# thedonutfactory/rs-tfhe

Hardware: AMD Instinct MI355X
Metric: gate-bootstraps/sec (hom_nand, SECURITY_128_BIT) (higher is better)
Workload: dtype f64

## Files before the change

rs-tfhe_amd/csrc/key_switch_mfma.hpp:

```cpp
#pragma once
#include <hip/hip_runtime.h>
#include <stdint.h>

#include <type_traits>

#include "experiment.hpp"

namespace tfhe {

#ifndef TFHE_KM_FRAGS
#define TFHE_KM_FRAGS 1
#endif
#ifndef TFHE_KM_COLBLOCKS
#define TFHE_KM_COLBLOCKS 2
#endif
constexpr int kKmWaves = 4;
constexpr int kKmFrags = TFHE_KM_FRAGS;
constexpr int kKmRows = 32 * kKmFrags * kKmWaves;
#ifndef TFHE_KM_SLOTS
#define TFHE_KM_SLOTS 4
#endif
constexpr int kKmSlots = TFHE_KM_SLOTS;
constexpr int kKmAhead = kKmSlots - 1;
constexpr int kKmAbBytes = 32 * kKmFrags * 16 * 4;
constexpr int kKmAbQ = kKmAbBytes / 256;
constexpr int kKmColBlocks = TFHE_KM_COLBLOCKS;
constexpr int kKmMaxTiles = 12 / kKmFrags;

__host__ __device__ constexpr int ks_mfma_tpw(int nt) { return (nt + kKmWaves - 1) / kKmWaves; }
__host__ __device__ constexpr int ks_mfma_slot_bytes(int nt) { return ks_mfma_tpw(nt) * kKmWaves * 1024; }
__host__ __device__ constexpr size_t ks_mfma_lds_bytes(int nt) {
  return (size_t)kKmSlots * ks_mfma_slot_bytes(nt) + (size_t)kKmWaves * 2 * kKmAbBytes + (size_t)kKmWaves * 256;
}
__host__ __device__ __forceinline__ int ks_mfma_total_tiles(int n) { return (n + 1 + 31) / 32; }
__host__ __device__ __forceinline__ int ks_mfma_tiles(int n) { return (ks_mfma_total_tiles(n) + kKmColBlocks - 1) / kKmColBlocks; }
__host__ __device__ __forceinline__ int ks_mfma_block_tiles(int n, int cb) {
  const int tiles = ks_mfma_total_tiles(n);
  return tiles / kKmColBlocks + (cb < tiles % kKmColBlocks ? 1 : 0);
}
__host__ __device__ __forceinline__ int ks_mfma_block_first(int n, int cb) {
  const int tiles = ks_mfma_total_tiles(n), base = tiles / kKmColBlocks, rem = tiles % kKmColBlocks;
  return cb * base + (cb < rem ? cb : rem);
}
__host__ __device__ __forceinline__ size_t ks_mfma_key_bytes(int n, int t) {
  return (size_t)4 * (64 * 2 * t) * ks_mfma_total_tiles(n) * 1024;
}
constexpr size_t kKmKeyTailPad = 64 * 1024;

__host__ __device__ __forceinline__ uint32_t ks_plane_byte(uint32_t w, int p) {
  uint32_t s = 0;
  for (int q = 0; q <= p; ++q) {
    s = w & 0xFFu;
    const uint32_t sext = (s & 0x80u) ? (s | 0xFFFFFF00u) : s;
    w = (w - sext) >> 8;
  }
  return s;
}

__global__ void k_ksk_planes(const uint32_t *__restrict__ eng, unsigned char *__restrict__ out, int n, int t,
                             size_t chunks) {
  const size_t idx = (size_t)blockIdx.x * blockDim.x + threadIdx.x;
  if (idx >= chunks) return;
  const int lane = (int)(idx & 63);
  size_t r = idx >> 6;
  const int S = 64 * 2 * t, tiles = ks_mfma_total_tiles(n);
  const size_t per_plane = (size_t)S * tiles;
  const int p = (int)(r / per_plane);
  r -= (size_t)p * per_plane;
  int cb = 0;
  while (cb + 1 < kKmColBlocks && r >= (size_t)S * ks_mfma_block_first(n, cb + 1)) ++cb;
  r -= (size_t)S * ks_mfma_block_first(n, cb);
  const int nt = ks_mfma_block_tiles(n, cb);
  const int s = (int)(r / (size_t)nt), c = (int)(r % (size_t)nt);
  const int col = (ks_mfma_block_first(n, cb) + c) * 32 + (lane & 31), kb = lane >> 5;
  const int blk = s / (2 * t), u = s % (2 * t), j = u >> 1, hh = u & 1;
  const int rw = (n + 1 + 3) & ~3;
  uint32_t o[4];
#pragma unroll
  for (int cc = 0; cc < 4; ++cc) {
    const int i = 16 * blk + 8 * hh + 4 * kb + cc;
    uint32_t d = 0;
#pragma unroll
    for (int k = 0; k < 4; ++k) {
      const size_t row = ((size_t)i * t + j) * 4 + k;
      const uint32_t w = (col <= n && k != 0) ? eng[row * (size_t)rw + col] : 0u;
      d |= ks_plane_byte(w, p) << (8 * k);
    }
    o[cc] = d;
  }
  reinterpret_cast<uint4 *>(out)[idx] = make_uint4(o[0], o[1], o[2], o[3]);
}

using km_i32x4 = __attribute__((ext_vector_type(4))) int;
using km_i32x16 = __attribute__((ext_vector_type(16))) int;
using km_u32x4 = __attribute__((ext_vector_type(4))) unsigned int;

__device__ __forceinline__ void km_dma16(uint32_t voff, const void *sbase, uint32_t lds) {
  uint32_t keep;
  asm volatile(
      "s_mov_b32 %0, m0\n\t"
      "s_mov_b32 m0, %3\n\t"
      "s_nop 0\n\t"
      "global_load_lds_dwordx4 %1, %2\n\t"
      "s_mov_b32 m0, %0"
      : "=&s"(keep)
      : "v"(voff), "s"(sbase), "s"(lds)
      : "memory");
}
__device__ __forceinline__ void km_dma4(uint32_t voff, const void *sbase, uint32_t lds) {
  uint32_t keep;
  asm volatile(
      "s_mov_b32 %0, m0\n\t"
      "s_mov_b32 m0, %3\n\t"
      "s_nop 0\n\t"
      "global_load_lds_dword %1, %2\n\t"
      "s_mov_b32 m0, %0"
      : "=&s"(keep)
      : "v"(voff), "s"(sbase), "s"(lds)
      : "memory");
}

struct KmPos {
  int blk, u;
};

#ifndef TFHE_KM_XCD
#define TFHE_KM_XCD 1
#endif
template <int NT>
__global__ __launch_bounds__(64 * kKmWaves, 2) void k_key_switch_mfma(const uint32_t *__restrict__ lv1,
                                                                       const unsigned char *__restrict__ ksk8,
                                                                       int n, int t, uint32_t *__restrict__ out,
                                                                       size_t count,
                                                                       unsigned long long *clk,
                                                                       int ksplit) {
  constexpr int N = 1024, D = kKmAhead, WAVES = kKmWaves, R = kKmFrags;
  constexpr int TPW = ks_mfma_tpw(NT), SLOT = ks_mfma_slot_bytes(NT), OPS = TPW + R;
  const unsigned long long clk0 = clk ? __builtin_amdgcn_s_memtime() : 0ull;
  const unsigned long long rtc0 = clk ? __builtin_amdgcn_s_memrealtime() : 0ull;
  extern __shared__ __attribute__((aligned(16))) unsigned char km_smem[];
  const int tid = threadIdx.x, lane = tid & 63;
  const int wave = __builtin_amdgcn_readfirstlane(tid >> 6);
  const uint32_t lds_base = (uint32_t)(size_t)(__attribute__((address_space(3))) unsigned char *)km_smem;
  const uint32_t off_ab = (uint32_t)(kKmSlots * SLOT) + (uint32_t)wave * 2u * kKmAbBytes;
  const uint32_t off_dump = (uint32_t)(kKmSlots * SLOT) + (uint32_t)(WAVES * 2 * kKmAbBytes) + (uint32_t)wave * 256u;
#if TFHE_KM_XCD
  const unsigned lin = blockIdx.x + gridDim.x * (blockIdx.y + gridDim.y * blockIdx.z);
  const unsigned combos = gridDim.y * gridDim.z, combo = lin % combos, rest = lin / combos;
  const int cb = (int)(combo % gridDim.y), plane = (int)(combo / gridDim.y);
#else
  const unsigned rest = blockIdx.x;
  const int cb = blockIdx.y, plane = blockIdx.z;
#endif
  const unsigned n_rb = gridDim.x / (unsigned)ksplit;
  const int kchunk = (int)(rest / n_rb);
  const int blk0 = kchunk * (64 / ksplit);
  const size_t row0 = (size_t)(rest % n_rb) * kKmRows + (size_t)wave * (32 * R);
  const int nt_blk = ks_mfma_block_tiles(n, cb), tile0 = ks_mfma_block_first(n, cb);
  const bool full = nt_blk == NT;
  const int spb = 2 * t, S = 64 * spb;
  const uint32_t prec = 1u << (31 - 2 * t);
  const uint32_t v16 = (uint32_t)lane * 16u;
  const uint32_t v4 = (uint32_t)(((lane >> 4) * (N + 1) + (lane & 15)) * 4);
  const uint32_t *ab_row0 = lv1 + row0 * (size_t)(N + 1);

  const unsigned char *kplane = ksk8 + ((size_t)plane * ks_mfma_total_tiles(n) + (size_t)tile0) * S * 1024;
  uint32_t koff[TPW];
#pragma unroll
  for (int i = 0; i < TPW; ++i) {
    const int tile = wave + i * WAVES;
    koff[i] = (uint32_t)(tile < nt_blk ? tile : nt_blk - 1) * 1024u + v16;
  }
  const uint32_t kstride = (uint32_t)nt_blk * 1024u;
  const int steps = S / ksplit;
#pragma unroll
  for (int i = 0; i < TPW; ++i) koff[i] += (uint32_t)(blk0 * spb) * kstride;
  auto dma_key = [&](uint32_t slot) {
#pragma unroll
    for (int i = 0; i < TPW; ++i) {
      km_dma16(koff[i], kplane, slot + (uint32_t)(wave + i * WAVES) * 1024u);
      koff[i] += kstride;
    }
  };

  for (int q = 0; q < kKmAbQ; ++q) km_dma4(v4, ab_row0 + (size_t)(4 * q) * (N + 1) + 16 * blk0, lds_base + off_ab + (uint32_t)q * 256u);
  for (int d = 0; d < D; ++d) dma_key(lds_base + (uint32_t)d * SLOT);
  asm volatile("s_waitcnt vmcnt(0)" ::: "memory");
  __builtin_amdgcn_s_barrier();
  asm volatile("" ::: "memory");

  km_i32x16 acc[R][NT];
  const uint32_t a_lane = (uint32_t)((lane & 31) * 64 + (lane >> 5) * 16);
  auto read_a = [&](const KmPos &q, int f) -> km_u32x4 {
    const unsigned char *abuf = km_smem + off_ab + (uint32_t)(q.blk & 1) * kKmAbBytes + a_lane + (uint32_t)(q.u & 1) * 32u;
    return *reinterpret_cast<const km_u32x4 *>(abuf + f * (32 * 64));
  };
  auto build_a = [&](const KmPos &q, km_u32x4 w) -> km_i32x4 {
    const uint32_t sh = (uint32_t)(27 - 2 * (q.u >> 1));
    km_u32x4 a;
    a.x = 1u << (((w.x + prec) >> sh) & 0x18u);
    a.y = 1u << (((w.y + prec) >> sh) & 0x18u);
    a.z = 1u << (((w.z + prec) >> sh) & 0x18u);
    a.w = 1u << (((w.w + prec) >> sh) & 0x18u);
    return __builtin_bit_cast(km_i32x4, a);
  };
  auto make_a = [&](const KmPos &q, int f) -> km_i32x4 { return build_a(q, read_a(q, f)); };
  KmPos cur{blk0, 0};
  km_i32x4 A[R];
#pragma unroll
  for (int f = 0; f < R; ++f) A[f] = make_a(cur, f);
#ifndef TFHE_KM_PRE
#define TFHE_KM_PRE 3
#endif
  constexpr int PRE = NT < TFHE_KM_PRE ? NT : TFHE_KM_PRE;
  constexpr int H = NT / 2;
  km_i32x4 Bpre[PRE];
#pragma unroll
  for (int c = 0; c < PRE; ++c) Bpre[c] = *reinterpret_cast<const km_i32x4 *>(km_smem + v16 + c * 1024);
#pragma unroll
  for (int f = 0; f < R; ++f)
#pragma unroll
    for (int c = 0; c < NT; ++c) acc[f][c] = km_i32x16{0, 0, 0, 0, 0, 0, 0, 0, 0, 0, 0, 0, 0, 0, 0, 0};
  auto run = [&](auto full_c) {
    constexpr bool FULL = decltype(full_c)::value;
#pragma unroll 1
    for (int g = 0; g < steps; ++g) {
      const unsigned char *slot = km_smem + (uint32_t)(g % kKmSlots) * SLOT + v16;
      const unsigned char *slot_next = km_smem + (uint32_t)((g + 1) % kKmSlots) * SLOT + v16;
      km_i32x4 B[NT];
#pragma unroll
      for (int c = 0; c < PRE; ++c) B[c] = Bpre[c];
#pragma unroll
      for (int c = 0; c < H; ++c) {
        if (c + PRE < NT) B[c + PRE] = *reinterpret_cast<const km_i32x4 *>(slot + (c + PRE) * 1024);
#pragma unroll
        for (int f = 0; f < R; ++f) acc[f][c] = __builtin_amdgcn_mfma_i32_32x32x32_i8(A[f], B[c], acc[f][c], 0, 0, 0);
      }
      __builtin_amdgcn_sched_barrier(0);
      asm volatile("s_waitcnt vmcnt(%0)" ::"n"((D - 2) * OPS) : "memory");
      if (!TFHE_ABL_KM_NOBARRIER) __builtin_amdgcn_s_barrier();
      asm volatile("" ::: "memory");
      const uint32_t dslot = lds_base + (uint32_t)((g + D) % kKmSlots) * SLOT;
      const int nblk = (cur.blk + 1) & 63;
      const uint32_t nbuf = lds_base + off_ab + (uint32_t)((cur.blk + 1) & 1) * kKmAbBytes;
      const int u_now = cur.u;
      constexpr int PIECES = TPW + R + 2;
      km_i32x4 A_next[R];
      km_u32x4 Aw[R];
      auto piece = [&](int it) {
        if (it == 0) {
          if (++cur.u == spb) {
            cur.u = 0;
            cur.blk = (cur.blk + 1) & 63;
          }
#pragma unroll
          for (int f = 0; f < R; ++f) Aw[f] = read_a(cur, f);
#pragma unroll
          for (int c = 0; c < PRE; ++c) Bpre[c] = *reinterpret_cast<const km_i32x4 *>(slot_next + c * 1024);
        } else if (it == PIECES - 2) {
#pragma unroll
          for (int f = 0; f < R; ++f) A_next[f] = build_a(cur, Aw[f]);
        } else {
          const int d = it - 1 - (it > PIECES - 2 ? 1 : 0);
          if (d < TPW) {
            km_dma16(koff[d], kplane, dslot + (uint32_t)(wave + d * WAVES) * 1024u);
            koff[d] += kstride;
          } else {
            const int q0 = R * u_now + (d - TPW);
            const uint32_t *s0 = ab_row0 + (size_t)(4 * (q0 & (kKmAbQ - 1))) * (N + 1) + 16 * nblk;
            km_dma4(v4, s0, q0 < kKmAbQ ? nbuf + (uint32_t)q0 * 256u : lds_base + off_dump);
          }
        }
      };
#pragma unroll
      for (int c = H; c < NT; ++c) {
        if (c + PRE < NT) B[c + PRE] = *reinterpret_cast<const km_i32x4 *>(slot + (c + PRE) * 1024);
        if (c < NT - 1 || FULL) {
#pragma unroll
          for (int f = 0; f < R; ++f) acc[f][c] = __builtin_amdgcn_mfma_i32_32x32x32_i8(A[f], B[c], acc[f][c], 0, 0, 0);
        }
        __builtin_amdgcn_sched_barrier(0);
        if (c - H < PIECES) piece(c - H);
        __builtin_amdgcn_sched_barrier(0);
      }
#pragma unroll
      for (int it = NT - H; it < PIECES; ++it) piece(it);
#pragma unroll
      for (int f = 0; f < R; ++f) A[f] = A_next[f];
    }
  };
  if (full)
    run(std::true_type{});
  else
    run(std::false_type{});
  {
    const int sh8 = 8 * plane;
    const int row_lim = (int)(count > row0 ? (count - row0 < 32 * R ? count - row0 : 32 * R) : 0) - 4 * (lane >> 5);
    const int col_lane = tile0 * 32 + (lane & 31);
    const uint32_t lane_off = (uint32_t)((4 * (lane >> 5)) * (n + 1) + col_lane) * 4u;
    unsigned char *obase = reinterpret_cast<unsigned char *>(out + row0 * (size_t)(n + 1));
    const uint32_t row_bytes = (uint32_t)(n + 1) * 4u;
#pragma unroll
    for (int f = 0; f < R; ++f)
#pragma unroll
      for (int c = 0; c < NT; ++c) {
        const bool col_ok = col_lane + 32 * c <= n && c < nt_blk;
        const bool is_body = col_lane + 32 * c == n && plane == 0 && kchunk == 0;
#pragma unroll
        for (int e = 0; e < 16; ++e) {
          const int er = 32 * f + (e & 3) + 8 * (e >> 2);
          if (col_ok && er < row_lim) {
            uint32_t v = 0u - ((uint32_t)acc[f][c][e] << sh8);
            if (is_body) v += lv1[(row0 + (size_t)(er + 4 * (lane >> 5))) * (size_t)(N + 1) + N];
            unsigned char *uni = obase + (size_t)((uint32_t)er * row_bytes + (uint32_t)(c * 128));
            if (v) atomicAdd(reinterpret_cast<uint32_t *>(uni + lane_off), v);
          }
        }
      }
  }
  asm volatile("s_waitcnt vmcnt(0)" ::: "memory");
  if (clk && tid == 0) {
    atomicAdd(&clk[0], __builtin_amdgcn_s_memtime() - clk0);
    atomicAdd(&clk[1], __builtin_amdgcn_s_memrealtime() - rtc0);
  }
}

}
```

Measured before the change: 191,000.

## Pack three nonzero key-switch digits per K slot to cut MFMA steps

After: 191,500 (median of 6 runs). Within noise of the previous version (+0.3%).

```diff
diff --git a/rs-tfhe_amd/csrc/key_switch_mfma.hpp b/rs-tfhe_amd/csrc/key_switch_mfma.hpp
--- a/rs-tfhe_amd/csrc/key_switch_mfma.hpp
+++ b/rs-tfhe_amd/csrc/key_switch_mfma.hpp
@@ -22,15 +22,16 @@
 #endif
 constexpr int kKmSlots = TFHE_KM_SLOTS;
 constexpr int kKmAhead = kKmSlots - 1;
-constexpr int kKmAbBytes = 32 * kKmFrags * 16 * 4;
+constexpr int kKmBlocks = 32;
+constexpr int kKmAbBytes = 32 * kKmFrags * 32 * 4;
 constexpr int kKmAbQ = kKmAbBytes / 256;
 constexpr int kKmColBlocks = TFHE_KM_COLBLOCKS;
 constexpr int kKmMaxTiles = 12 / kKmFrags;
 
 __host__ __device__ constexpr int ks_mfma_tpw(int nt) { return (nt + kKmWaves - 1) / kKmWaves; }
-__host__ __device__ constexpr int ks_mfma_slot_bytes(int nt) { return ks_mfma_tpw(nt) * kKmWaves * 1024; }
+__host__ __device__ constexpr int ks_mfma_slot_bytes(int nt) { return nt * 1024; }
 __host__ __device__ constexpr size_t ks_mfma_lds_bytes(int nt) {
-  return (size_t)kKmSlots * ks_mfma_slot_bytes(nt) + (size_t)kKmWaves * 2 * kKmAbBytes + (size_t)kKmWaves * 256;
+  return (size_t)kKmSlots * ks_mfma_slot_bytes(nt) + (size_t)kKmWaves * 2 * kKmAbBytes + 1024;
 }
 __host__ __device__ __forceinline__ int ks_mfma_total_tiles(int n) { return (n + 1 + 31) / 32; }
 __host__ __device__ __forceinline__ int ks_mfma_tiles(int n) { return (ks_mfma_total_tiles(n) + kKmColBlocks - 1) / kKmColBlocks; }
@@ -42,8 +43,9 @@
   const int tiles = ks_mfma_total_tiles(n), base = tiles / kKmColBlocks, rem = tiles % kKmColBlocks;
   return cb * base + (cb < rem ? cb : rem);
 }
+__host__ __device__ __forceinline__ int ks_mfma_steps(int t) { return kKmBlocks * 3 * t; }
 __host__ __device__ __forceinline__ size_t ks_mfma_key_bytes(int n, int t) {
-  return (size_t)4 * (64 * 2 * t) * ks_mfma_total_tiles(n) * 1024;
+  return (size_t)4 * ks_mfma_steps(t) * ks_mfma_total_tiles(n) * 1024;
 }
 constexpr size_t kKmKeyTailPad = 64 * 1024;
 
@@ -63,7 +65,7 @@
   if (idx >= chunks) return;
   const int lane = (int)(idx & 63);
   size_t r = idx >> 6;
-  const int S = 64 * 2 * t, tiles = ks_mfma_total_tiles(n);
+  const int S = ks_mfma_steps(t), tiles = ks_mfma_total_tiles(n);
   const size_t per_plane = (size_t)S * tiles;
   const int p = (int)(r / per_plane);
   r -= (size_t)p * per_plane;
@@ -73,20 +75,21 @@
   const int nt = ks_mfma_block_tiles(n, cb);
   const int s = (int)(r / (size_t)nt), c = (int)(r % (size_t)nt);
   const int col = (ks_mfma_block_first(n, cb) + c) * 32 + (lane & 31), kb = lane >> 5;
-  const int blk = s / (2 * t), u = s % (2 * t), j = u >> 1, hh = u & 1;
+  const int unit = s / 3, s3 = s % 3, blk = unit / t, j = unit % t;
   const int rw = (n + 1 + 3) & ~3;
   uint32_t o[4];
 #pragma unroll
-  for (int cc = 0; cc < 4; ++cc) {
-    const int i = 16 * blk + 8 * hh + 4 * kb + cc;
-    uint32_t d = 0;
-#pragma unroll
-    for (int k = 0; k < 4; ++k) {
+  for (int d = 0; d < 4; ++d) {
+    uint32_t v = 0;
+#pragma unroll
+    for (int e = 0; e < 4; ++e) {
+      const int B = 16 * s3 + 4 * d + e;
+      const int i = 32 * blk + 16 * kb + B / 3, k = B % 3 + 1;
       const size_t row = ((size_t)i * t + j) * 4 + k;
-      const uint32_t w = (col <= n && k != 0) ? eng[row * (size_t)rw + col] : 0u;
-      d |= ks_plane_byte(w, p) << (8 * k);
+      const uint32_t w = col <= n ? eng[row * (size_t)rw + col] : 0u;
+      v |= ks_plane_byte(w, p) << (8 * e);
     }
-    o[cc] = d;
+    o[d] = v;
   }
   reinterpret_cast<uint4 *>(out)[idx] = make_uint4(o[0], o[1], o[2], o[3]);
 }
@@ -121,7 +124,7 @@
 }
 
 struct KmPos {
-  int blk, u;
+  int blk, j;
 };
 
 #ifndef TFHE_KM_XCD
@@ -136,6 +139,7 @@
                                                                        int ksplit) {
   constexpr int N = 1024, D = kKmAhead, WAVES = kKmWaves, R = kKmFrags;
   constexpr int TPW = ks_mfma_tpw(NT), SLOT = ks_mfma_slot_bytes(NT), OPS = TPW + R;
+  static_assert(kKmBlocks * 32 == N, "a block is the 32 coefficients of one unit");
   const unsigned long long clk0 = clk ? __builtin_amdgcn_s_memtime() : 0ull;
   const unsigned long long rtc0 = clk ? __builtin_amdgcn_s_memrealtime() : 0ull;
   extern __shared__ __attribute__((aligned(16))) unsigned char km_smem[];
@@ -143,7 +147,7 @@
   const int wave = __builtin_amdgcn_readfirstlane(tid >> 6);
   const uint32_t lds_base = (uint32_t)(size_t)(__attribute__((address_space(3))) unsigned char *)km_smem;
   const uint32_t off_ab = (uint32_t)(kKmSlots * SLOT) + (uint32_t)wave * 2u * kKmAbBytes;
-  const uint32_t off_dump = (uint32_t)(kKmSlots * SLOT) + (uint32_t)(WAVES * 2 * kKmAbBytes) + (uint32_t)wave * 256u;
+  const uint32_t off_dump = (uint32_t)(kKmSlots * SLOT) + (uint32_t)(WAVES * 2 * kKmAbBytes);
 #if TFHE_KM_XCD
   const unsigned lin = blockIdx.x + gridDim.x * (blockIdx.y + gridDim.y * blockIdx.z);
   const unsigned combos = gridDim.y * gridDim.z, combo = lin % combos, rest = lin / combos;
@@ -154,61 +158,93 @@
 #endif
   const unsigned n_rb = gridDim.x / (unsigned)ksplit;
   const int kchunk = (int)(rest / n_rb);
-  const int blk0 = kchunk * (64 / ksplit);
+  const int blk0 = kchunk * (kKmBlocks / ksplit);
   const size_t row0 = (size_t)(rest % n_rb) * kKmRows + (size_t)wave * (32 * R);
   const int nt_blk = ks_mfma_block_tiles(n, cb), tile0 = ks_mfma_block_first(n, cb);
   const bool full = nt_blk == NT;
-  const int spb = 2 * t, S = 64 * spb;
+  const int spb = 3 * t, S = kKmBlocks * spb;
   const uint32_t prec = 1u << (31 - 2 * t);
   const uint32_t v16 = (uint32_t)lane * 16u;
-  const uint32_t v4 = (uint32_t)(((lane >> 4) * (N + 1) + (lane & 15)) * 4);
+  const uint32_t v4row = (uint32_t)((lane >> 4) * (N + 1) * 4), v4col = (uint32_t)((lane & 15) * 4);
   const uint32_t *ab_row0 = lv1 + row0 * (size_t)(N + 1);
+  auto dma_ab = [&](int q, int blk, uint32_t dst) {
+    const int qq = q & (kKmAbQ - 1);
+    const uint32_t *s0 = ab_row0 + (size_t)(32 * (qq >> 4) + 4 * (qq & 7)) * (N + 1) + 32 * blk + 16 * ((qq >> 3) & 1);
+    km_dma4(v4row + (v4col ^ ((uint32_t)(qq & 3) << 4)), s0, dst);
+  };
 
   const unsigned char *kplane = ksk8 + ((size_t)plane * ks_mfma_total_tiles(n) + (size_t)tile0) * S * 1024;
   uint32_t koff[TPW];
+  uint32_t kdst[TPW];
+  bool kin[TPW];
 #pragma unroll
   for (int i = 0; i < TPW; ++i) {
     const int tile = wave + i * WAVES;
     koff[i] = (uint32_t)(tile < nt_blk ? tile : nt_blk - 1) * 1024u + v16;
+    kin[i] = tile < NT;
+    kdst[i] = kin[i] ? (uint32_t)tile * 1024u : off_dump;
   }
   const uint32_t kstride = (uint32_t)nt_blk * 1024u;
   const int steps = S / ksplit;
 #pragma unroll
   for (int i = 0; i < TPW; ++i) koff[i] += (uint32_t)(blk0 * spb) * kstride;
-  auto dma_key = [&](uint32_t slot) {
-#pragma unroll
-    for (int i = 0; i < TPW; ++i) {
-      km_dma16(koff[i], kplane, slot + (uint32_t)(wave + i * WAVES) * 1024u);
-      koff[i] += kstride;
-    }
-  };
-
-  for (int q = 0; q < kKmAbQ; ++q) km_dma4(v4, ab_row0 + (size_t)(4 * q) * (N + 1) + 16 * blk0, lds_base + off_ab + (uint32_t)q * 256u);
-  for (int d = 0; d < D; ++d) dma_key(lds_base + (uint32_t)d * SLOT);
+  auto dma_key_piece = [&](int i, uint32_t slot_off) {
+    const bool in_slot = (i + 1) * WAVES <= NT || kin[i];
+    km_dma16(koff[i], kplane, lds_base + (in_slot ? slot_off : 0u) + kdst[i]);
+    koff[i] += kstride;
+  };
+
+  for (int q = 0; q < kKmAbQ; ++q) dma_ab(q, blk0, lds_base + off_ab + (uint32_t)q * 256u);
+  for (int d = 0; d < D; ++d)
+#pragma unroll
+    for (int i = 0; i < TPW; ++i) dma_key_piece(i, (uint32_t)d * SLOT);
   asm volatile("s_waitcnt vmcnt(0)" ::: "memory");
   __builtin_amdgcn_s_barrier();
   asm volatile("" ::: "memory");
 
   km_i32x16 acc[R][NT];
-  const uint32_t a_lane = (uint32_t)((lane & 31) * 64 + (lane >> 5) * 16);
-  auto read_a = [&](const KmPos &q, int f) -> km_u32x4 {
-    const unsigned char *abuf = km_smem + off_ab + (uint32_t)(q.blk & 1) * kKmAbBytes + a_lane + (uint32_t)(q.u & 1) * 32u;
-    return *reinterpret_cast<const km_u32x4 *>(abuf + f * (32 * 64));
-  };
-  auto build_a = [&](const KmPos &q, km_u32x4 w) -> km_i32x4 {
-    const uint32_t sh = (uint32_t)(27 - 2 * (q.u >> 1));
+  const uint32_t a_lane = (uint32_t)((lane >> 5) * 2048 + (lane & 31) * 64 + (((lane >> 2) & 3) << 4));
+  struct KmAw {
+    km_u32x4 lo, hi;
+  };
+  auto read_a = [&](const KmPos &q, int s3, int f) -> KmAw {
+    const unsigned char *abuf = km_smem + off_ab + (uint32_t)(q.blk & 1) * kKmAbBytes + f * 4096;
+    KmAw w;
+    w.lo = *reinterpret_cast<const km_u32x4 *>(abuf + (a_lane ^ ((uint32_t)s3 << 4)));
+    w.hi = *reinterpret_cast<const km_u32x4 *>(abuf + (a_lane ^ ((uint32_t)(s3 + 1) << 4)));
+    return w;
+  };
+  constexpr uint32_t P1 = 0x05030201u, P2 = 0x06050302u, P3 = 0x07060503u;
+  auto build_a = [&](const KmPos &q, auto s3c, const KmAw &w) -> km_i32x4 {
+    constexpr int S3 = decltype(s3c)::value;
+    const uint32_t sh = (uint32_t)(27 - 2 * q.j);
+    const uint32_t ww[8] = {w.lo.x, w.lo.y, w.lo.z, w.lo.w, w.hi.x, w.hi.y, w.hi.z, w.hi.w};
+    uint32_t o[6];
+#pragma unroll
+    for (int c = 0; c < 6; ++c) o[c] = 1u << (((ww[S3 + c] + prec) >> sh) & 0x18u);
     km_u32x4 a;
-    a.x = 1u << (((w.x + prec) >> sh) & 0x18u);
-    a.y = 1u << (((w.y + prec) >> sh) & 0x18u);
-    a.z = 1u << (((w.z + prec) >> sh) & 0x18u);
-    a.w = 1u << (((w.w + prec) >> sh) & 0x18u);
+    if constexpr (S3 == 0) {
+      a.x = __builtin_amdgcn_perm(o[1], o[0], P1);
+      a.y = __builtin_amdgcn_perm(o[2], o[1], P2);
+      a.z = __builtin_amdgcn_perm(o[3], o[2], P3);
+      a.w = __builtin_amdgcn_perm(o[5], o[4], P1);
+    } else if constexpr (S3 == 1) {
+      a.x = __builtin_amdgcn_perm(o[1], o[0], P2);
+      a.y = __builtin_amdgcn_perm(o[2], o[1], P3);
+      a.z = __builtin_amdgcn_perm(o[4], o[3], P1);
+      a.w = __builtin_amdgcn_perm(o[5], o[4], P2);
+    } else {
+      a.x = __builtin_amdgcn_perm(o[1], o[0], P3);
+      a.y = __builtin_amdgcn_perm(o[3], o[2], P1);
+      a.z = __builtin_amdgcn_perm(o[4], o[3], P2);
+      a.w = __builtin_amdgcn_perm(o[5], o[4], P3);
+    }
     return __builtin_bit_cast(km_i32x4, a);
   };
-  auto make_a = [&](const KmPos &q, int f) -> km_i32x4 { return build_a(q, read_a(q, f)); };
   KmPos cur{blk0, 0};
   km_i32x4 A[R];
 #pragma unroll
-  for (int f = 0; f < R; ++f) A[f] = make_a(cur, f);
+  for (int f = 0; f < R; ++f) A[f] = build_a(cur, std::integral_constant<int, 0>{}, read_a(cur, 0, f));
 #ifndef TFHE_KM_PRE
 #define TFHE_KM_PRE 3
 #endif
@@ -223,8 +259,8 @@
     for (int c = 0; c < NT; ++c) acc[f][c] = km_i32x16{0, 0, 0, 0, 0, 0, 0, 0, 0, 0, 0, 0, 0, 0, 0, 0};
   auto run = [&](auto full_c) {
     constexpr bool FULL = decltype(full_c)::value;
-#pragma unroll 1
-    for (int g = 0; g < steps; ++g) {
+    auto step = [&](auto s3c, int g) {
+      constexpr int S3 = decltype(s3c)::value, S3N = (S3 + 1) % 3;
       const unsigned char *slot = km_smem + (uint32_t)(g % kKmSlots) * SLOT + v16;
       const unsigned char *slot_next = km_smem + (uint32_t)((g + 1) % kKmSlots) * SLOT + v16;
       km_i32x4 B[NT];
@@ -240,36 +276,31 @@
       asm volatile("s_waitcnt vmcnt(%0)" ::"n"((D - 2) * OPS) : "memory");
       if (!TFHE_ABL_KM_NOBARRIER) __builtin_amdgcn_s_barrier();
       asm volatile("" ::: "memory");
-      const uint32_t dslot = lds_base + (uint32_t)((g + D) % kKmSlots) * SLOT;
-      const int nblk = (cur.blk + 1) & 63;
+      const uint32_t dslot = (uint32_t)((g + D) % kKmSlots) * SLOT;
+      const int nblk = (cur.blk + 1) & (kKmBlocks - 1);
       const uint32_t nbuf = lds_base + off_ab + (uint32_t)((cur.blk + 1) & 1) * kKmAbBytes;
-      const int u_now = cur.u;
+      const int u_now = 3 * cur.j + S3;
       constexpr int PIECES = TPW + R + 2;
       km_i32x4 A_next[R];
-      km_u32x4 Aw[R];
+      KmAw Aw[R];
       auto piece = [&](int it) {
         if (it == 0) {
-          if (++cur.u == spb) {
-            cur.u = 0;
-            cur.blk = (cur.blk + 1) & 63;
+          if (S3 == 2 && ++cur.j == t) {
+            cur.j = 0;
+            cur.blk = (cur.blk + 1) & (kKmBlocks - 1);
           }
 #pragma unroll
-          for (int f = 0; f < R; ++f) Aw[f] = read_a(cur, f);
+          for (int f = 0; f < R; ++f) Aw[f] = read_a(cur, S3N, f);
 #pragma unroll
           for (int c = 0; c < PRE; ++c) Bpre[c] = *reinterpret_cast<const km_i32x4 *>(slot_next + c * 1024);
-        } else if (it == PIECES - 2) {
-#pragma unroll
-          for (int f = 0; f < R; ++f) A_next[f] = build_a(cur, Aw[f]);
+        } else if (it <= TPW) {
+          dma_key_piece(it - 1, dslot);
+        } else if (it == TPW + 1) {
+#pragma unroll
+          for (int f = 0; f < R; ++f) A_next[f] = build_a(cur, std::integral_constant<int, S3N>{}, Aw[f]);
         } else {
-          const int d = it - 1 - (it > PIECES - 2 ? 1 : 0);
-          if (d < TPW) {
-            km_dma16(koff[d], kplane, dslot + (uint32_t)(wave + d * WAVES) * 1024u);
-            koff[d] += kstride;
-          } else {
-            const int q0 = R * u_now + (d - TPW);
-            const uint32_t *s0 = ab_row0 + (size_t)(4 * (q0 & (kKmAbQ - 1))) * (N + 1) + 16 * nblk;
-            km_dma4(v4, s0, q0 < kKmAbQ ? nbuf + (uint32_t)q0 * 256u : lds_base + off_dump);
-          }
+          const int q0 = R * u_now + (it - TPW - 2);
+          dma_ab(q0, nblk, q0 < kKmAbQ ? nbuf + (uint32_t)q0 * 256u : lds_base + off_dump + (uint32_t)wave * 256u);
         }
       };
 #pragma unroll
@@ -279,14 +310,20 @@
 #pragma unroll
           for (int f = 0; f < R; ++f) acc[f][c] = __builtin_amdgcn_mfma_i32_32x32x32_i8(A[f], B[c], acc[f][c], 0, 0, 0);
         }
-        __builtin_amdgcn_sched_barrier(0);
+        if (c - H <= TPW + 1) __builtin_amdgcn_sched_barrier(0);
         if (c - H < PIECES) piece(c - H);
-        __builtin_amdgcn_sched_barrier(0);
+        if (c - H <= TPW) __builtin_amdgcn_sched_barrier(0);
       }
 #pragma unroll
       for (int it = NT - H; it < PIECES; ++it) piece(it);
 #pragma unroll
       for (int f = 0; f < R; ++f) A[f] = A_next[f];
+    };
+#pragma unroll 1
+    for (int g = 0; g < steps; g += 3) {
+      step(std::integral_constant<int, 0>{}, g);
+      step(std::integral_constant<int, 1>{}, g + 1);
+      step(std::integral_constant<int, 2>{}, g + 2);
     }
   };
   if (full)
```
